# swacisko/ALGA

Measured on AMD Instinct MI355X. Metric: overlap_edges_per_sec, higher is better.
Workload: dtype u32; 1 GPU; cfg4_50M_150bp: 50000000 x 150 bp reads, genome 250000000, seed 11, err 0.00 -> 90621096 nodes (both strands, duplicates removed), min_overlap 82, rsoemo 116; generated on the device (alga_amd.workload.device_build) in 1.0 s; nodes=90621096, edges=92350115

## Files before the change

### alga_amd/csrc/engine.hip

```cpp
#include <hip/hip_runtime.h>

#include <algorithm>
#include <chrono>
#include <cstdio>
#include <cstdlib>
#include <cstring>
#include <new>
#include <string>
#include <thread>
#include <vector>

#include "engine_internal.h"

using namespace alga;

namespace {

using Prepared = AlgaPrepared;

int prepare(alga_engine *e, const alga_nodes *nodes, const alga_prefsuf_params *p, hipStream_t s, Prepared &out) {
    if (!nodes || !p) return alga_fail(e, ALGA_ERR_INVALID_ARGUMENT, "nodes/params must not be NULL");
    if (nodes->n < 0) return alga_fail(e, ALGA_ERR_INVALID_ARGUMENT, "negative node count");
    if (nodes->n > 0 && (!nodes->words || !nodes->len)) return alga_fail(e, ALGA_ERR_INVALID_ARGUMENT, "words/len must not be NULL");
    if (nodes->stride_words <= 0 && nodes->n > 0) return alga_fail(e, ALGA_ERR_INVALID_ARGUMENT, "stride_words must be positive");
// ... 417 lines not shown
                            (unsigned long long *) e->seg_val.p, n_rec, bits, s));
    launch_rowptr_from_sorted((const uint32_t *) e->seg_key.p, cnt + CNT_SORT_VALID, n_rec, n_owned, (uint32_t *) e->rowptr.p, s);
    if ((rc = alga_check_launch(e, "k_rowptr_from_sorted"))) return rc;
    launch_gather_heads(nd, (const unsigned long long *) e->seg_val.p, cnt + CNT_SORT_VALID, n_rec, e->heads.p, s);
    if ((rc = alga_check_launch(e, "k_gather_heads"))) return rc;
    HIP_TRY(e, hipEventRecord(e->ev[EV_GROUP], s));

    if ((rc = alga_ensure(e, e->out_cnt, (size_t) (n_owned + 1) * sizeof(uint32_t)))) return rc;
    if ((rc = alga_ensure(e, e->outdeg, (size_t) (nd.n + 1) * sizeof(uint32_t)))) return rc;
    HIP_TRY(e, hipMemsetAsync(e->outdeg.p, 0, (size_t) (nd.n + 1) * sizeof(uint32_t), s));
    const int tpb = reduce_targets_per_block(n_valid_hint, (uint64_t) std::max(1, n_owned));
    launch_reduce_targets(nd, cfg, dst_begin, n_owned, tpb, (const uint32_t *) e->rowptr.p, (unsigned long long *) e->seg_val.p,
                          e->heads.p, (uint32_t *) e->out_cnt.p, (uint32_t *) e->outdeg.p, cnt, s);
    if ((rc = alga_check_launch(e, "k_reduce_targets"))) return rc;
    HIP_TRY(e, hipEventRecord(e->ev[EV_REDUCE], s));

    if ((rc = alga_ensure(e, e->scan_scratch, scan_scratch_bytes((uint64_t) nd.n)))) return rc;
    if ((rc = alga_ensure(e, e->out_rowptr, (size_t) (nd.n + 1) * sizeof(uint32_t)))) return rc;
    launch_exclusive_scan((const uint32_t *) e->outdeg.p, (uint64_t) nd.n, (uint32_t *) e->out_rowptr.p, (uint64_t *) e->scan_scratch.p, s);
    if ((rc = alga_check_launch(e, "scan(outdeg)"))) return rc;
    uint64_t *d_total = (uint64_t *) e->scan_scratch.p + scan_total_index((uint64_t) nd.n);
    HIP_TRY(e, hipMemcpyAsync(&e->h_counters[CNT_TOTAL], d_total, sizeof(uint64_t), hipMemcpyDeviceToHost, s));
    HIP_TRY(e, hipMemcpyAsync(e->h_counters, cnt, CNT_TOTAL * sizeof(unsigned long long), hipMemcpyDeviceToHost, s));
    HIP_TRY(e, hipStreamSynchronize(s));
    const uint64_t E = e->h_counters[CNT_TOTAL];
    if (E >= (1ull << 32) - 16) return alga_fail(e, ALGA_ERR_CAPACITY, "more than 2^32 edges; shard the input");
    if ((rc = alga_ensure(e, e->edges, (size_t) (E + 1) * sizeof(alga_edge_dev)))) return rc;
    launch_scatter_by_source(cfg, dst_begin, n_owned, (const uint32_t *) e->rowptr.p, (const unsigned long long *) e->seg_val.p,
                             (const uint32_t *) e->out_cnt.p, (const uint32_t *) e->out_rowptr.p, (uint32_t *) e->outdeg.p,
                             (alga_edge_dev *) e->edges.p, s);
    if ((rc = alga_check_launch(e, "k_scatter_by_source"))) return rc;
    launch_sort_rows(nd.n, (const uint32_t *) e->out_rowptr.p, (alga_edge_dev *) e->edges.p, s);
    if ((rc = alga_check_launch(e, "k_sort_rows"))) return rc;
    HIP_TRY(e, hipEventRecord(e->ev[EV_EMIT], s));
    HIP_TRY(e, hipStreamSynchronize(s));
    *n_edges = E;
    e->stats.edges = E;
    e->stats.transitive_listed = e->h_counters[CNT_TR_LISTED];
    e->stats.transitive_compares = e->h_counters[CNT_TR_COMPARES];
    e->stats.transitive_removed = e->h_counters[CNT_TR_REMOVED];
    e->stats.max_in_records = e->h_counters[CNT_MAX_IN];
    return ALGA_OK;
}

int finalize_local(alga_engine *e, const Prepared &pp, int32_t src_begin, int32_t src_end, uint64_t n_rec, hipStream_t s, uint64_t *n_edges) {
    int rc;
    *n_edges = 0;
    const uint64_t n_src = (uint64_t) std::max<int64_t>(0, (int64_t) src_end - src_begin);
    if ((rc = alga_ensure(e, e->scan_scratch, scan_scratch_bytes(n_src)))) return rc;
    if ((rc = alga_ensure(e, e->out_rowptr, (size_t) (n_src + 1) * sizeof(uint32_t)))) return rc;
    if ((rc = alga_ensure(e, e->out_cnt, (size_t) (n_src + 1) * sizeof(uint32_t)))) return rc;
    HIP_TRY(e, hipEventRecord(e->ev[EV_GROUP], s));
    HIP_TRY(e, hipEventRecord(e->ev[EV_REDUCE], s));
    if (e->pile_deg_pending)
        launch_exclusive_scan_pile_deg((uint32_t *) e->outdeg.p, n_src, (uint32_t *) e->out_rowptr.p, (uint64_t *) e->scan_scratch.p, (unsigned long long *) e->loc_first.p,
                                       (const unsigned long long *) e->cl_pile_cnt.p, s);
    else
        launch_exclusive_scan((const uint32_t *) e->outdeg.p, n_src, (uint32_t *) e->out_rowptr.p, (uint64_t *) e->scan_scratch.p, s);
    e->pile_deg_pending = false;
    if ((rc = alga_check_launch(e, "scan(outdeg)"))) return rc;
    const uint64_t E = e->stats.records;
    if (E >= (1ull << 32) - 16) return alga_fail(e, ALGA_ERR_CAPACITY, "more than 2^32 edges; shard the input");
    if ((rc = alga_ensure(e, e->edges, (size_t) (E + 1) * sizeof(alga_edge_dev)))) return rc;
    launch_local_emit(src_begin, (int32_t) n_src, (const uint32_t *) e->outdeg.p, (const unsigned long long *) e->loc_first.p,
                      e->loc_second_used ? (const unsigned long long *) e->loc_second.p : nullptr, (const uint32_t *) e->rec_dst.p, (const unsigned long long *) e->rec_val.p, n_rec, (const uint32_t *) e->out_rowptr.p,
                      (uint32_t *) e->out_cnt.p, (alga_edge_dev *) e->edges.p,
                      e->defer_list_valid ? (const int32_t *) e->cl_defer.p : nullptr, (const unsigned long long *) e->counters.p + CNT_DEFERRED, (uint32_t) n_src, s,
                      e->loc_second_used ? e->loc_slot_stride : 0u);
    if ((rc = alga_check_launch(e, "k_local_emit"))) return rc;
    HIP_TRY(e, hipEventRecord(e->ev[EV_EMIT], s));
    uint64_t *d_total = (uint64_t *) e->scan_scratch.p + scan_total_index(n_src);
    HIP_TRY(e, hipMemcpyAsync(&e->h_counters[CNT_TOTAL], d_total, sizeof(uint64_t), hipMemcpyDeviceToHost, s));
    HIP_TRY(e, hipStreamSynchronize(s));
    if (e->h_counters[CNT_TOTAL] != E) return alga_fail(e, ALGA_ERR_HIP, "source-side emit: out-degrees and edge count disagree");
    *n_edges = E;
    e->stats.edges = E;
    return ALGA_OK;
}

int build_local(alga_engine *e, const Prepared &pp, int32_t src_begin, int32_t src_end, hipStream_t s, uint64_t *n_edges) {
    if (!pp.local_ok) return alga_fail(e, ALGA_ERR_UNSUPPORTED, "source-side reduction is not exact for this input (read lengths / masks / rsoemo)");
    uint64_t n_rec = 0;
    bool overflow = false;
    int rc = discover_impl(e, pp, src_begin, src_end, s, &n_rec, true, &overflow);
    if (rc) return rc;
    if (overflow) return alga_fail(e, ALGA_ERR_UNSUPPORTED, "a source node has more raw overlaps than the source-side reduction holds");
    if ((rc = finalize_local(e, pp, src_begin, src_end, n_rec, s, n_edges))) return rc;
    e->stats.reduction_used = ALGA_REDUCTION_SOURCE_SIDE;
    return ALGA_OK;
}

double now_ms_host() { return std::chrono::duration<double, std::milli>(std::chrono::steady_clock::now().time_since_epoch()).count(); }

float ev_ms(alga_engine *e, int a, int b) {
    float ms = 0.f;
    if (hipEventElapsedTime(&ms, e->ev[a], e->ev[b]) != hipSuccess) return 0.f;
    return ms;
}

void store_phase_stats(alga_engine *e) {
    if (!e->store_timed) return;
    e->stats.ms_keys = ev_ms(e, EV_START, EV_KEYS);
    e->stats.ms_sort = ev_ms(e, EV_KEYS, EV_SORT);
    e->stats.ms_dir = ev_ms(e, e->dir_late ? EV_SAMPLE : EV_SORT, EV_DIR);
    e->stats.ms_gather = ev_ms(e, EV_DIR, EV_GATHER) + (e->dir_late ? ev_ms(e, EV_SORT, EV_SAMPLE) : 0.0);
    e->stats.ms_pile = e->pile_timed ? ev_ms(e, EV_GATHER, EV_SEED) : 0.0;
}

}

int alga_prepare(alga_engine *e, const alga_nodes *nodes, const alga_prefsuf_params *p, hipStream_t s, AlgaPrepared &out) { return prepare(e, nodes, p, s, out); }
int alga_cluster_alloc(alga_engine *e, const AlgaPrepared &pp) { return cluster_alloc(e, pp); }

extern "C" {

int alga_abi_version(void) { return ALGA_AMD_ABI_VERSION; }

struct DeviceGuard {
    int prev = -1;
    DeviceGuard() { if (hipGetDevice(&prev) != hipSuccess) prev = -1; }
    ~DeviceGuard() { if (prev >= 0) (void) hipSetDevice(prev); }
// ... 38 lines not shown
    if (rc != ALGA_OK) { engine_free_handles(e); delete e; return rc; }
    *out = e;
    return ALGA_OK;
}

void alga_engine_destroy(alga_engine *e) {
    if (!e) return;
    DeviceGuard guard;
    (void) hipSetDevice(e->device);
    if (e->own_stream) (void) hipStreamSynchronize(e->own_stream);
    if (e->side_stream) (void) hipStreamSynchronize(e->side_stream);
    for (DevBuf *b : e->owned) alga_release(*b);
    alga_release(e->up_raw);
    for (DevBuf *b : {&e->in_bytes[0], &e->in_bytes[1], &e->in_nl[0], &e->in_nl[1], &e->in_tiles, &e->in_tile_off}) alga_release(*b);
    for (DevBuf *b : {&e->sp_rowptr, &e->sp_sorted, &e->sp_list, &e->sp_cnt, &e->sp_orow, &e->sp_out, &e->sp_in}) alga_release(*b);
    alga_staging_release(e);
    for (void *&p : e->gfa_pin) { if (p) (void) hipHostFree(p); p = nullptr; }
    for (auto &kv : e->host_lists) free(kv.first);
    e->host_lists.clear();
    engine_free_handles(e);
    delete e;
}

const char *alga_last_error(const alga_engine *e) { return e ? e->err.c_str() : "no engine"; }

int alga_engine_device_name(const alga_engine *e, char *buf, size_t buflen) {
    if (!e || !buf || buflen == 0) return ALGA_ERR_INVALID_ARGUMENT;
    snprintf(buf, buflen, "%s", e->dev_name);
    return ALGA_OK;
}

int alga_engine_set_option(alga_engine *e, const char *name, int64_t value) {
    if (!e || !name) return ALGA_ERR_INVALID_ARGUMENT;
    e->err.clear();
    if (!strcmp(name, "probe")) {
        if (value < ALGA_PROBE_AUTO || value > ALGA_PROBE_CLUSTER) return alga_fail(e, ALGA_ERR_INVALID_ARGUMENT, "option probe: 0 auto, 1 table, 2 cluster");
        e->opt_probe = (int) value;
    } else if (!strcmp(name, "cluster_bucket_bias")) {
        if (value < -8 || value > 8) return alga_fail(e, ALGA_ERR_INVALID_ARGUMENT, "option cluster_bucket_bias: -8 .. 8");
        e->opt_cluster_bucket_bias = (int) value;
    } else if (!strcmp(name, "cluster_pairs")) {
        e->opt_cluster_pairs = value != 0;
    } else if (!strcmp(name, "pile")) {
        e->opt_pile = (value == 2 || value == 3) ? (int) value : (value != 0);
    } else if (!strcmp(name, "pile_runs")) {
        e->opt_pile_runs = value != 0;
    } else if (!strcmp(name, "pile_runs_list")) {
        e->opt_pile_runs_list = value != 0;
    } else if (!strcmp(name, "pile_dir")) {
        if (value < 0 || value > 2) return alga_fail(e, ALGA_ERR_INVALID_ARGUMENT, "option pile_dir: 0 directory records, 1 k_pile_build from the keys, 2 ... and no directory for a pure pile build");
        e->opt_pile_dir = (int) value;
    } else if (!strcmp(name, "pile_deg_fold")) {
        e->opt_pile_deg_fold = value != 0;
    } else if (!strcmp(name, "pile_probe_lean")) {
        e->opt_pile_probe_lean = value != 0;
    } else if (!strcmp(name, "pile_stream_by_id")) {
        e->opt_pile_stream_by_id = value != 0;
    } else if (!strcmp(name, "pile_check")) {
        e->opt_pile_check = value != 0;
    } else if (!strcmp(name, "pile_skip_gather")) {
        e->opt_pile_skip_gather = value != 0;
    } else if (!strcmp(name, "cluster_order")) {
        e->opt_cluster_order = value != 0;
    } else if (!strcmp(name, "local_big_max")) {
        e->big_limit = value < 0 ? -1 : (int) std::min<int64_t>(value, 1 << 20);
    } else if (!strcmp(name, "shard_bucket_max")) {
        e->opt_shard_dmax = (int) std::max<int64_t>(1, std::min<int64_t>(value, 4096));
    } else if (!strcmp(name, "rsort_variant")) {
        rsort_set_variant((int) value);
    } else if (!strcmp(name, "stream_slots")) {
        e->opt_stream_slots = value >= 4 ? 4 : 2;
    } else if (!strcmp(name, "pile_range")) {
        e->opt_pile_range = value != 0;
    } else if (!strcmp(name, "pkb_legacy")) {
        e->opt_pkb_legacy = (int) value;
    } else if (!strcmp(name, "own_sort")) {
        e->opt_own_sort = value != 0;
    } else if (!strcmp(name, "test_presort_oom")) {
        e->opt_test_presort_oom = value != 0;
    } else if (!strcmp(name, "test_pile_oom")) {
        e->opt_test_pile_oom = value != 0;
    } else if (!strcmp(name, "test_unsorted_index")) {
        e->opt_test_unsorted_index = value != 0;
    } else if (!strcmp(name, "gfa_chunk_mb")) {
        if (value < 1 || value > 4096) return alga_fail(e, ALGA_ERR_INVALID_ARGUMENT, "option gfa_chunk_mb: 1 .. 4096");
        e->opt_gfa_chunk_mb = (int) value;
    } else if (!strcmp(name, "mst_mid_nodes")) {
        if (value < 8 || value > (1 << 20)) return alga_fail(e, ALGA_ERR_INVALID_ARGUMENT, "option mst_mid_nodes: 8 .. 2^20");
        e->opt_mst_mid_nodes = (int) value;
    } else if (!strcmp(name, "consensus_max_blocks")) {
        if (value < 0 || value > (1 << 20)) return alga_fail(e, ALGA_ERR_INVALID_ARGUMENT, "option consensus_max_blocks: 0 .. 2^20");
        e->opt_consensus_max_blocks = (int) value;
    } else if (!strcmp(name, "unitig_ruling")) {
        if (value < -1 || value > 1) return alga_fail(e, ALGA_ERR_INVALID_ARGUMENT, "option unitig_ruling: -1, 0 or 1");
        e->opt_unitig_ruling = (int) value;
    } else if (!strcmp(name, "correct_slice_keys")) {
        if (value < 1 || value > (1ll << 31)) return alga_fail(e, ALGA_ERR_INVALID_ARGUMENT, "option correct_slice_keys: 1 .. 2^31");
        e->opt_correct_slice_keys = value;
    } else if (!strcmp(name, "correct_dir_bits")) {
        if (value < 0 || value > 28) return alga_fail(e, ALGA_ERR_INVALID_ARGUMENT, "option correct_dir_bits: 0 (auto) or 1 .. 28");
        e->opt_correct_dir_bits = (int) value;
    } else if (!strcmp(name, "place_dir_bits")) {
        if (value < 0 || value > 26) return alga_fail(e, ALGA_ERR_INVALID_ARGUMENT, "option place_dir_bits: 0 (auto) or 1 .. 26");
        e->opt_place_dir_bits = (int) value;
    } else if (!strcmp(name, "auto_reduction_per_target")) {
        e->opt_force_per_target = value != 0;
// ... 668 lines not shown
```

### alga_amd/csrc/engine_internal.h

```cpp
#pragma once
#include <hip/hip_runtime.h>

#include <cstdio>
#include <algorithm>
#include <string>
#include <vector>
#include <unordered_map>

#include "../../include/alga_amd.h"
#include "prefsuf_common.h"
#include "prefsuf_kernels.h"
#include "pkb_kernels.h"

struct DevBuf {
    void  *p = nullptr;
    size_t cap = 0;
};

enum { EV_START = 0, EV_SEED, EV_PROBE, EV_GROUP, EV_REDUCE, EV_EMIT, EV_PAIRS, EV_KEYS, EV_SORT, EV_GATHER, EV_DIR, EV_SAMPLE, EV_COUNT };
constexpr int ALGA_STAGE_THREADS = 8;

struct alga_engine {
    std::vector<DevBuf *> owned;
    int         device = -1;
    hipStream_t own_stream = nullptr;
    hipStream_t side_stream = nullptr;
    hipEvent_t  ev_side = nullptr;
    std::string err;
    char        dev_name[256] = {0};
    int         n_cu = 256;
    int         seed_fill_x10 = 20;
    int         opt_probe = 0;
    int         opt_cluster_bucket_bias = 0;
    int         opt_force_per_target = 0;
    int         opt_shard_dmax = 4096;
    int         opt_test_unsorted_index = 0;
    hipEvent_t  ev[EV_COUNT] = {};
    DevBuf table, filter, counters, rowptr, rec_dst, rec_val, keys, seg_key, seg_val, heads, sort_temp, out_cnt, outdeg, out_rowptr, edges, scan_scratch;
    DevBuf cl_defer;
    uint32_t h_first_hkey = 255;
    int32_t keyed_n = -1, keyed_begin = 0, keyed_end = 0;
    bool defer_list_valid = false;
    const void *keyed_words = nullptr;
    int32_t store_n = -1, store_run_begin = 0, store_run_end = 0, store_eq = 0;
    uint32_t store_buckets = 0;
    const void *store_words = nullptr;
    int stat_max_len = 0, stat_min_len = 0; uint64_t stat_live = 0; unsigned long long stat_mask_asym = 0;
    const void *stat_len = nullptr, *stat_from = nullptr, *stat_to = nullptr;
    bool   warmed = false;
    bool   pairs_timed = false;
    bool   store_timed = false;
    bool   pile_keys_only = false, pile_kept_pure = false;
    int    opt_pile_range = 1;
    int    opt_pile_skip_gather = 1;
    int    opt_pile = 1;
    int    opt_pile_runs = 1;
    int    opt_pile_runs_list = 1;
    DevBuf cl_pile_list;
    int    opt_pile_deg_fold = 1;
    int    opt_pile_dir = 2;
    bool   dir_late = false;
    bool   pile_tab_index = false;
    int    opt_pile_stream_by_id = 0;
    int    opt_pile_probe_lean = 1;
    bool   pile_deg_pending = false;
    int    opt_pile_check = 0;
    bool   expect_pairwise = false;
    DevBuf cl_pile_side_r, cl_pile_cursor;
    DevBuf cl_pile_own;
    int    opt_pkb_legacy = 0;
    int    opt_own_sort = 1;
    int    opt_test_presort_oom = 0;
    int    opt_test_pile_oom = 0;
    bool   pile_timed = false;
    DevBuf cl_pile_succ;
    DevBuf cl_pile_rec2;
    DevBuf cl_pile_rec, cl_pile_cnt, cl_pile_tab;
    uint32_t pile_epoch = 0;
    int32_t pile_n = -1; const void *pile_words = nullptr;
    int    opt_cluster_order = 1;
    int    opt_cluster_pairs = 1;
    DevBuf cl_keys[2], cl_vals[2], cl_meta, cl_runs, cl_nruns, cl_store, cl_dir;
    DevBuf loc_second;
    bool   loc_second_used = false;
    uint32_t loc_slot_stride = 0;
    int    opt_stream_slots = 4;
    DevBuf loc_first, loc_big_list, loc_big_items;
    int    big_limit = -1;
    DevBuf edge_keys, edge_keys2, edge_vals, edge_vals2, edges_sorted, xs_dst, xs_val;
    DevBuf up_words, up_len, up_from, up_to;
    DevBuf up_len_narrow;
    DevBuf cp_deg, cp_dst, cp_off;
    DevBuf cl_defer2;
    DevBuf pk_keys, pk_keys2, pk_vals, pk_vals2, pk_marks, pk_big, pk_add, pk_ekeys, pk_ekeys2, pk_flag, pk_pos, pk_edges[2], pk_rowptr, pk_deg,
           pk_mask, pk_cnt, pk_io, pk_io2, pk_tips, pk_heads, pk_g[2], pk_addk, pk_addk2, pk_merged, pk_hsz, pk_hsz2, pk_heads2, pk_nadd, pk_koff,
           pk_gsz, pk_fixlist, pk_bounds, pk_tiprec, pk_tipidx, pk_keys_all, pk_vals_all;
    DevBuf pk_keys2b, pk_vals2b, pk_headsb, pk_hszb, sort_temp2, pk_fixlist2, pk_cnt2;
    DevBuf pp_rows, pp_len, pp_perm[2], pp_keys[2], pp_mark, pp_keep, pp_pos, pp_out_rows, pp_out_len, pp_out_pair, pp_tally;
    bool        stage_ready = false;
    void       *stage_pin[ALGA_STAGE_THREADS][2] = {};
    hipEvent_t  stage_ev[ALGA_STAGE_THREADS][2] = {};
    hipStream_t stage_stream[ALGA_STAGE_THREADS] = {};
    DevBuf      up_raw;
    std::unordered_map<void *, size_t> host_lists;
    void       *host_spare = nullptr;
    size_t      host_spare_cap = 0;
    DevBuf      in_bytes[2], in_nl[2], in_tiles, in_tile_off;
    DevBuf      sp_rowptr, sp_sorted, sp_list, sp_cnt, sp_orow, sp_out, sp_in;
    DevBuf      tp_cnt, tp_keys[2], tp_vals[2], tp_flag, tp_pos, tp_best, tp_est, tp_rev, tp_rfid, tp_rowptr[2], tp_alive, tp_kill, tp_rec[2], tp_branch,
                tp_overflow, tp_ws, tp_out;
    DevBuf      mp_cnt, mp_rowptr, mp_rows, mp_len, mp_owner, mp_pend[2], mp_win, mp_overflow, mp_overflow2, mp_ws, mp_ws_big, mp_orow, mp_out;
    struct MstFilled { const void *p = nullptr; size_t bytes = 0; uint32_t hbits = 0, cap_nodes = 0, cap_edges = 0; int32_t n_ws = 0; } mp_filled[2];
// ... 195 lines not shown
```

### alga_amd/csrc/prefsuf_kernels.h

```cpp
#pragma once
#include <hip/hip_runtime.h>
#include <stddef.h>
#include <stdint.h>
#include "prefsuf_common.h"

namespace alga {

struct alga_edge_dev { int32_t src, dst, offset; };

void launch_restride(const uint32_t *in, int stride_in, uint32_t *out, int stride_out, uint64_t n, hipStream_t s);
void launch_widen_len(const void *in, int elem_bytes , int32_t *out, uint64_t n, hipStream_t s);
void launch_compact_edges(const alga_edge_dev *edges, int32_t n, uint64_t n_edges, uint8_t *deg, uint32_t *dst, uint8_t *off, unsigned long long *bad, hipStream_t s);
void launch_expand_twins(const uint32_t *in, int stride_in, const int32_t *len , uint32_t *out, int stride_out, uint64_t n_pairs, hipStream_t s);
void launch_node_stats(const NodesDev &nd, unsigned long long *counters, int *max_len , hipStream_t s);

uint32_t seed_buckets_for(uint64_t live_nodes, int fill_x10);
uint32_t seed_filter_bits_for(uint64_t live_nodes);
void launch_seed_build(const NodesDev &nd, const PrefSufCfg &cfg, unsigned long long *table, uint32_t n_buckets, uint32_t *filter,
                       uint32_t filter_bits, hipStream_t s);

struct ProbeBig { int32_t *list; uint32_t list_cap; uint32_t count; void *items; uint32_t item_cap; };
int    local_item_capacity();
int    local_big_limit();
size_t probe_big_bytes(int n_cu, uint32_t count, int local, uint32_t item_cap);

void launch_probe(const NodesDev &nd, const PrefSufCfg &cfg, const unsigned long long *table, uint32_t n_buckets,
                  const uint32_t *filter, uint32_t filter_bits, int32_t src_begin, int32_t src_end, uint32_t *rec_dst, unsigned long long *rec_val, uint64_t rec_cap,
                  unsigned long long *counters, int n_cu, int local , uint32_t *deg , unsigned long long *first ,
                  const ProbeBig *big , hipStream_t s);
uint64_t probe_record_slack(int n_cu, uint64_t n_src, bool local);
void launch_local_emit(int32_t src_base, int32_t n_src, const uint32_t *deg, const unsigned long long *first, const unsigned long long *second,
                       const uint32_t *rec_dst, const unsigned long long *rec_val, uint64_t n_rec, const uint32_t *rowptr, uint32_t *cursor,
                       alga_edge_dev *edges, const int32_t *record_sources, const unsigned long long *record_sources_count, uint32_t record_sources_cap, hipStream_t s, uint32_t slot_stride = 0);

bool       cluster_plan(const PrefSufCfg &cfg, int max_len, uint64_t live, int bucket_log2_bias, ClusterCfg *c, int *eq);
size_t     cluster_sort_temp_bytes(uint64_t n);
void       launch_cluster_keys(const NodesDev &nd, const PrefSufCfg &cfg, const ClusterCfg &cc, int32_t node_begin, int32_t node_end, uint32_t *keys,
                               uint32_t *vals, uint32_t *meta, void *runs, uint8_t *nruns, hipStream_t s, bool with_runs = true ,
                               const unsigned long long *only_if_declined = nullptr );
void       launch_cluster_runs_list(const NodesDev &nd, const PrefSufCfg &cfg, const ClusterCfg &cc, const int32_t *ids, const unsigned long long *count, uint32_t cap,
                                    uint32_t grid_blocks, void *runs, uint8_t *nruns, hipStream_t s);
hipError_t launch_cluster_store(const NodesDev &nd, const ClusterCfg &cc, uint32_t *keys, uint32_t *vals, uint32_t *keys2 , uint32_t *vals2, void *sort_temp,
                                size_t sort_temp_bytes, void *dir, bool fill_vals, hipEvent_t ev_sorted ,
                                unsigned long long *bad_flag ,
                                bool test_skip_sort , hipStream_t s, bool own_sort = true);
hipError_t launch_cluster_sort(const NodesDev &nd, const ClusterCfg &cc, uint32_t *keys, uint32_t *vals, uint32_t *keys2, uint32_t *vals2, void *sort_temp, size_t sort_temp_bytes,
                               bool fill_vals, hipEvent_t ev_sorted, bool test_skip_sort, hipStream_t s, bool own_sort = true);
hipError_t launch_cluster_dir(const NodesDev &nd, const ClusterCfg &cc, const uint32_t *keys2, void *dir, unsigned long long *bad_flag, const unsigned long long *only_if_no_pure_piles,
                              hipStream_t s);
hipError_t launch_cluster_gather(const NodesDev &nd, const ClusterCfg &cc, int eq, const uint32_t *keys2, const uint32_t *vals2, const uint32_t *meta,
                                 int uniform_len , void *store,
                                 const unsigned long long *pile_cnt , hipStream_t s);
uint64_t   cluster_record_slack(int n_cu, uint64_t n_src);
void       launch_probe_clustered(const NodesDev &nd, const PrefSufCfg &cfg, const ClusterCfg &cc, int eq, const void *store, const void *dir,
                                  const void *runs, const uint8_t *nruns, int32_t src_begin, int32_t src_end, const int32_t *src_list, int32_t src_base, uint32_t *rec_dst, unsigned long long *rec_val, uint64_t rec_cap,
                                  unsigned long long *counters, int n_cu, uint32_t *deg, unsigned long long *first, const ProbeBig *big,
                                  const unsigned long long *list_count ,
                                  int sw , hipStream_t s,
                                  const uint32_t *skeys = nullptr, const uint32_t *sids = nullptr, int uniform_len = 0,
                                  const unsigned long long *pile_cnt = nullptr ,
                                  const void *tab = nullptr , uint32_t epoch = 0);
void       launch_probe_stream(const NodesDev &nd, const PrefSufCfg &cfg, const ClusterCfg &cc, int eq, const void *store, const void *dir,
                               const void *runs, const uint8_t *nruns, int32_t src_begin, int32_t src_end, bool by_key ,
                               unsigned long long *counters, int n_cu, uint32_t *deg, unsigned long long *first, unsigned long long *second, int32_t *defer_list,
                               uint32_t defer_cap, const unsigned long long *pile_cnt ,
                               hipStream_t s, uint32_t slot_stride = 0 );
void       launch_pile_deg(int32_t n, unsigned long long *first, uint32_t *deg, const unsigned long long *pile_cnt, hipStream_t s);
bool       pile_plan(const PrefSufCfg &cfg, const ClusterCfg &cc, int eq, int uniform_len, bool masks);
size_t     pile_record_bytes(uint64_t n);
size_t     pile_table_bytes(uint32_t n_buckets);
void       launch_pile_sample(const NodesDev &nd, const ClusterCfg &cc, int uniform_len, const uint32_t *skeys , const uint32_t *sids , const void *dir,
                              unsigned long long *pile_cnt , int no_sample, hipStream_t s,
                              bool from_keys = false );
constexpr int PILE_CNT_WORDS = 6;
size_t     pile_own_mask_bytes(uint64_t n);
size_t     pile_list_bytes(uint64_t n);
void       launch_pile_build(const NodesDev &nd, const PrefSufCfg &cfg, const ClusterCfg &cc, int uniform_len, const uint32_t *skeys, const uint32_t *sids, const void *dir, void *rec,
                             void *rec2 , void *tab, uint32_t epoch, void *side, const void *runs, int nwin, const unsigned long long *pile_cnt,
                             uint32_t *own_mask ,
                             void *plist , hipStream_t s,
                             bool from_keys = false , unsigned long long *bad_flag = nullptr,
                             bool full_record = false );
void       launch_pile_own_ids(const uint32_t *own_mask, const uint32_t *sids, uint64_t n_entries, int32_t *list, uint32_t cap, unsigned long long *pile_cnt, hipStream_t s);
void       launch_pile_check(const void *side, uint64_t n_entries, uint32_t n_buckets, const void *tab, const void *rec2, uint32_t epoch, const void *runs, int n_nodes, int nwin,
                             unsigned long long *pile_cnt, hipStream_t s);
bool       launch_probe_stream_list(const NodesDev &nd, const PrefSufCfg &cfg, const ClusterCfg &cc, int eq, const void *store, const void *dir, const void *runs, const uint8_t *nruns,
// ... 67 lines not shown
```

### alga_amd/csrc/prefsuf_kernels.hip

```cpp
#include <hip/hip_runtime.h>
#include <algorithm>
#include "prefsuf_common.h"
#include "prefsuf_kernels.h"
#include "prefsuf_device.h"
#include "prefsuf_cluster_device.h"

namespace alga {

__global__ void __launch_bounds__(256) k_node_stats(NodesDev nd, unsigned long long *counters, int *max_len) {
    __shared__ int s_max[4], s_min[4];
    __shared__ unsigned long long s_live[4];
    int m = 0, mn = 0x7FFFFFFF;
    unsigned long long live = 0, asym = 0;
    auto one = [&](int l, int64_t i) {
        m = l > m ? l : m;
        mn = (l > 0 && l < mn) ? l : mn;
        live += l > 0;
        if (nd.to && l > 0 && !nd.to[i] && (nd.from == nullptr || nd.from[i])) asym++;
    };
    const int64_t gid = (int64_t) blockIdx.x * blockDim.x + threadIdx.x, gsz = (int64_t) gridDim.x * blockDim.x;
    int64_t done = 0;
    if ((reinterpret_cast<uintptr_t>(nd.len) & 15u) == 0) {
        const int64_t nq = (int64_t) nd.n >> 2;
        const int4 *len4 = reinterpret_cast<const int4 *>(nd.len);
// ... 834 lines not shown
            atomicMax(&counters[CNT_MAX_IN], (unsigned long long) mk);
        }
    }
}

__global__ void __launch_bounds__(256)
k_scatter_by_source(PrefSufCfg cfg, int32_t dst_begin, int32_t n_owned, const uint32_t *__restrict__ rowptr,
                    const unsigned long long *__restrict__ seg_val, const uint32_t *__restrict__ out_cnt,
                    const uint32_t *__restrict__ out_rowptr, uint32_t *__restrict__ out_cursor, alga_edge_dev *__restrict__ edges) {
    const int t = blockIdx.x * blockDim.x + threadIdx.x;
    if (t >= n_owned) return;
    const uint32_t beg = rowptr[t], cnt = out_cnt[t];
    const int C = dst_begin + t;
    for (uint32_t u = 0; u < cnt; u++) {
        const unsigned long long v = seg_val[beg + u];
        const int A = (int) (uint32_t) v;
        const int off = ol_off((uint32_t) (v >> 32));
        const int row = cfg.reversed ? C : A;
        const int col = cfg.reversed ? A : C;
        const uint32_t pos = out_rowptr[row] + (atomicSub(&out_cursor[row], 1u) - 1u);
        edges[pos].src = row; edges[pos].dst = col; edges[pos].offset = off;
    }
}

__global__ void __launch_bounds__(256)
k_sort_rows(int32_t n, const uint32_t *__restrict__ out_rowptr, alga_edge_dev *__restrict__ edges) {
    const int a = blockIdx.x * blockDim.x + threadIdx.x;
    if (a >= n) return;
    const uint32_t beg = out_rowptr[a], k = out_rowptr[a + 1] - beg;
    alga_edge_dev *e = edges + beg;
    for (uint32_t i = 1; i < k; i++) {
        const alga_edge_dev x = e[i];
        uint32_t j = i;
        while (j > 0 && (e[j - 1].dst > x.dst || (e[j - 1].dst == x.dst && e[j - 1].offset > x.offset))) { e[j] = e[j - 1]; j--; }
        e[j] = x;
    }
}

__global__ void __launch_bounds__(256) k_edges_to_keys(const alga_edge_dev *__restrict__ e, uint64_t n, unsigned long long *__restrict__ keys,
                                                        uint32_t *__restrict__ vals) {
    for (uint64_t i = (uint64_t) blockIdx.x * blockDim.x + threadIdx.x; i < n; i += (uint64_t) gridDim.x * blockDim.x) {
        keys[i] = ((unsigned long long) (uint32_t) e[i].src << 32) | (uint32_t) e[i].dst;
        vals[i] = (uint32_t) e[i].offset;
    }
}

__global__ void __launch_bounds__(256) k_keys_to_edges(const unsigned long long *__restrict__ keys, const uint32_t *__restrict__ vals, uint64_t n,
                                                        alga_edge_dev *__restrict__ e) {
    for (uint64_t i = (uint64_t) blockIdx.x * blockDim.x + threadIdx.x; i < n; i += (uint64_t) gridDim.x * blockDim.x) {
        e[i].src = (int32_t) (keys[i] >> 32); e[i].dst = (int32_t) (uint32_t) keys[i]; e[i].offset = (int32_t) vals[i];
    }
}

__global__ void __launch_bounds__(256) k_local_emit_first(int32_t src_base, int32_t n_src, const uint32_t *__restrict__ deg,
                                                           const unsigned long long *__restrict__ first, const unsigned long long *__restrict__ second,
                                                           const uint32_t *__restrict__ rowptr, alga_edge_dev *__restrict__ edges, uint32_t slot_stride) {
    const int i = blockIdx.x * blockDim.x + threadIdx.x;
    if (i >= n_src) return;
    const uint32_t dg = deg[i];
    if (dg == 0) return;
    const unsigned long long f = first[i];
    if (f == LOCAL_FIRST_NONE) return;
    alga_edge_dev e;
    e.src = src_base + i; e.dst = (int32_t) (uint32_t) (f >> 32); e.offset = (int32_t) (uint32_t) f;
    const uint32_t at = rowptr[i];
    edges[at] = e;
    if (dg >= 3u && dg <= (uint32_t) LOCAL_SLOTS_MAX && second != nullptr && slot_stride != 0u) {
        unsigned long long k[LOCAL_SLOTS_MAX];
        k[0] = f;
#pragma unroll
        for (int q = 1; q < LOCAL_SLOTS_MAX; q++) k[q] = (uint32_t) q < dg ? second[(size_t) (q - 1) * slot_stride + (size_t) i] : ~0ull;
#pragma unroll
        for (int a = 0; a < LOCAL_SLOTS_MAX; a++)
#pragma unroll
            for (int b = (a & 1); b + 1 < LOCAL_SLOTS_MAX; b += 2) { const unsigned long long lo = min(k[b], k[b + 1]), hi = max(k[b], k[b + 1]); k[b] = lo; k[b + 1] = hi; }
#pragma unroll
        for (int q = 0; q < LOCAL_SLOTS_MAX; q++)
            if ((uint32_t) q < dg) { alga_edge_dev x; x.src = src_base + i; x.dst = (int32_t) (uint32_t) (k[q] >> 32); x.offset = (int32_t) (uint32_t) k[q]; edges[at + q] = x; }
        return;
    }
    if (dg == 2u && second != nullptr) {
        const unsigned long long g = second[i];
        alga_edge_dev e2 = e;
        e2.dst = (int32_t) (uint32_t) (g >> 32); e2.offset = (int32_t) (uint32_t) g;
        if (e2.dst < e.dst || (e2.dst == e.dst && e2.offset < e.offset)) { edges[at] = e2; e2 = e; }
        edges[at + 1] = e2;
    }
}

__global__ void __launch_bounds__(256) k_zero_cursors_list(const int32_t *__restrict__ list, const unsigned long long *__restrict__ count, uint32_t cap, int32_t src_base,
                                                            uint32_t *__restrict__ cursor) {
    unsigned long long m = *count;
    if (m > (unsigned long long) cap) m = cap;
    for (unsigned long long q = (unsigned long long) blockIdx.x * blockDim.x + threadIdx.x; q < m; q += (unsigned long long) gridDim.x * blockDim.x) cursor[list[q] - src_base] = 0u;
}

__global__ void __launch_bounds__(256) k_sort_rows_list(const int32_t *__restrict__ list, const unsigned long long *__restrict__ count, uint32_t cap, int32_t src_base,
                                                         const uint32_t *__restrict__ out_rowptr, alga_edge_dev *__restrict__ edges) {
    unsigned long long m = *count;
    if (m > (unsigned long long) cap) m = cap;
    for (unsigned long long q = (unsigned long long) blockIdx.x * blockDim.x + threadIdx.x; q < m; q += (unsigned long long) gridDim.x * blockDim.x) {
        const int a = list[q] - src_base;
        const uint32_t beg = out_rowptr[a], k = out_rowptr[a + 1] - beg;
        alga_edge_dev *e = edges + beg;
        for (uint32_t i = 1; i < k; i++) {
            const alga_edge_dev x = e[i];
            uint32_t j = i;
            while (j > 0 && (e[j - 1].dst > x.dst || (e[j - 1].dst == x.dst && e[j - 1].offset > x.offset))) { e[j] = e[j - 1]; j--; }
            e[j] = x;
        }
    }
}

__global__ void __launch_bounds__(256) k_local_emit_records(int32_t src_base, const uint32_t *__restrict__ rec_dst,
                                                             const unsigned long long *__restrict__ rec_val, uint64_t n_rec,
                                                             const uint32_t *__restrict__ rowptr, uint32_t *__restrict__ cursor,
                                                             alga_edge_dev *__restrict__ edges) {
    for (uint64_t i = (uint64_t) blockIdx.x * blockDim.x + threadIdx.x; i < n_rec; i += (uint64_t) gridDim.x * blockDim.x) {
        const uint32_t c = rec_dst[i];
        if (c == REC_INVALID) continue;
        const unsigned long long v = rec_val[i];
        const int32_t src = (int32_t) (uint32_t) v;
        alga_edge_dev e;
        e.src = src; e.dst = (int32_t) c; e.offset = ol_off((uint32_t) (v >> 32));
        edges[rowptr[src - src_base] + atomicAdd(&cursor[src - src_base], 1u)] = e;
    }
}

__global__ void __launch_bounds__(256) k_restride(const uint32_t *__restrict__ in, int stride_in, uint32_t *__restrict__ out, int stride_out, uint64_t n) {
    const uint64_t total = n * (uint64_t) stride_out;
    for (uint64_t i = (uint64_t) blockIdx.x * blockDim.x + threadIdx.x; i < total; i += (uint64_t) gridDim.x * blockDim.x) {
        const uint64_t r = i / (uint64_t) stride_out;
        const int c = (int) (i - r * (uint64_t) stride_out);
        out[i] = c < stride_in ? in[r * (uint64_t) stride_in + c] : 0u;
    }
}

__device__ __forceinline__ uint32_t nuc_revcomp32(uint32_t x) {
    x = __brev(x);
    x = ((x >> 1) & 0x55555555u) | ((x & 0x55555555u) << 1);
// ... 116 lines not shown
struct ProbeTable { const unsigned long long *table; uint32_t n_buckets; const uint32_t *filter; uint32_t filter_mask; };

template <int NQ, int LOCAL>
static void launch_probe_nql(const NodesDev &nd, const PrefSufCfg &cfg, const ProbeTable &t,
                             int32_t src_begin, int32_t src_end, const ProbeOut &o, dim3 grid, dim3 block, hipStream_t s) {
    if constexpr (LOCAL != 0) {
        if (o.big_count) {
            hipLaunchKernelGGL((k_probe_sources<true, NQ, LOCAL, true>), grid, block, 0, s, nd, cfg, t.table, t.n_buckets, t.filter, t.filter_mask, src_begin, src_end, o);
            return;
        }
    }
    if (cfg.stats) hipLaunchKernelGGL((k_probe_sources<true, NQ, LOCAL>), grid, block, 0, s, nd, cfg, t.table, t.n_buckets, t.filter, t.filter_mask, src_begin, src_end, o);
    else           hipLaunchKernelGGL((k_probe_sources<false, NQ, LOCAL>), grid, block, 0, s, nd, cfg, t.table, t.n_buckets, t.filter, t.filter_mask, src_begin, src_end, o);
}
template <int NQ>
static void launch_probe_nq(const NodesDev &nd, const PrefSufCfg &cfg, const ProbeTable &t, int local,
                            int32_t src_begin, int32_t src_end, const ProbeOut &o, dim3 grid, dim3 block, hipStream_t s) {
    if (local == 1)      launch_probe_nql<NQ, 1>(nd, cfg, t, src_begin, src_end, o, grid, block, s);
    else if (local == 2) launch_probe_nql<NQ, 2>(nd, cfg, t, src_begin, src_end, o, grid, block, s);
    else                 launch_probe_nql<NQ, 0>(nd, cfg, t, src_begin, src_end, o, grid, block, s);
}

void launch_probe(const NodesDev &nd, const PrefSufCfg &cfg, const unsigned long long *table, uint32_t n_buckets,
                  const uint32_t *filter, uint32_t filter_bits,
                  int32_t src_begin, int32_t src_end, uint32_t *rec_dst, unsigned long long *rec_val, uint64_t rec_cap,
                  unsigned long long *counters, int n_cu, int local, uint32_t *deg, unsigned long long *first, const ProbeBig *big, hipStream_t s) {
    const int64_t ns = (int64_t) src_end - src_begin;
    if (ns <= 0) return;
    const bool second = local && big && big->count > 0;
    dim3 grid((unsigned) probe_blocks(n_cu, second ? (uint64_t) big->count : (uint64_t) ns)), block(PROBE_WAVES * 64);
    ProbeOut o{rec_dst, rec_val, rec_cap, counters, deg, first, src_begin};
    if (local && big) {
        o.big_list = big->list; o.big_list_cap = big->list_cap;
        if (second) {
            const size_t items = (size_t) grid.x * PROBE_WAVES * (size_t) big->item_cap;
            o.big_count = big->count;
            o.bigO = (uint4 *) big->items;
            o.bigC = (uint32_t *) (o.bigO + items * (size_t) local);
            o.bigM = o.bigC + items;
            o.big_cap = big->item_cap;
        }
    }
    ProbeTable t{table, n_buckets, filter_bits ? filter : nullptr, filter_bits ? filter_bits - 1 : 0u};
    const int need_q = (((2 * cfg.Lcap + 31) >> 5) + 3) >> 2;
    const bool aligned = (nd.stride & 3) == 0 && ((uintptr_t) nd.words & 15u) == 0;
    const int row_q = nd.stride >> 2;
    if (aligned && need_q <= 2 && row_q >= 2)      launch_probe_nq<2>(nd, cfg, t, local, src_begin, src_end, o, grid, block, s);
    else if (aligned && need_q <= 3 && row_q >= 3) launch_probe_nq<3>(nd, cfg, t, local, src_begin, src_end, o, grid, block, s);
    else if (aligned && need_q <= 4 && row_q >= 4) launch_probe_nq<4>(nd, cfg, t, local, src_begin, src_end, o, grid, block, s);
    else                                           launch_probe_nq<0>(nd, cfg, t, local, src_begin, src_end, o, grid, block, s);
}

void launch_local_emit(int32_t src_base, int32_t n_src, const uint32_t *deg, const unsigned long long *first, const unsigned long long *second,
                       const uint32_t *rec_dst, const unsigned long long *rec_val, uint64_t n_rec, const uint32_t *rowptr, uint32_t *cursor,
                       alga_edge_dev *edges, const int32_t *record_sources, const unsigned long long *record_sources_count, uint32_t record_sources_cap, hipStream_t s,
                       uint32_t slot_stride) {
    if (n_src <= 0) return;
    if (record_sources) hipLaunchKernelGGL(k_zero_cursors_list, dim3(std::min<unsigned>(grid_for((uint64_t) record_sources_cap, 256), 2048u)), dim3(256), 0, s, record_sources, record_sources_count,
                                           record_sources_cap, src_base, cursor);
    else (void) hipMemsetAsync(cursor, 0, (size_t) (n_src + 1) * sizeof(uint32_t), s);
    hipLaunchKernelGGL(k_local_emit_first, dim3(grid_for((uint64_t) n_src, 256)), dim3(256), 0, s, src_base, n_src, deg, first, second, rowptr, edges, slot_stride);
    if (n_rec) {
        unsigned g = std::min<unsigned>(grid_for(n_rec, 256), 4096u);
        hipLaunchKernelGGL(k_local_emit_records, dim3(std::max(1u, g)), dim3(256), 0, s, src_base, rec_dst, rec_val, n_rec, rowptr, cursor, edges);
    }
    if (record_sources) {
        if (n_rec) hipLaunchKernelGGL(k_sort_rows_list, dim3(std::min<unsigned>(grid_for((uint64_t) record_sources_cap, 256), 2048u)), dim3(256), 0, s, record_sources, record_sources_count,
                                      record_sources_cap, src_base, rowptr, edges);
    } else hipLaunchKernelGGL(k_sort_rows, dim3(grid_for((uint64_t) n_src, 256)), dim3(256), 0, s, n_src, rowptr, edges);
}

void launch_make_keys(const uint32_t *rec_dst, uint64_t n_rec, int32_t dst_begin, int32_t dst_end, uint32_t *keys,
                      unsigned long long *n_valid, hipStream_t s) {
    if (n_rec == 0) return;
    unsigned g = std::min<unsigned>(grid_for(n_rec, 256 * 4), 4096u);
    hipLaunchKernelGGL(k_make_keys, dim3(std::max(1u, g)), dim3(256), 0, s, rec_dst, n_rec, dst_begin, dst_end, keys, n_valid);
}

void launch_rowptr_from_sorted(const uint32_t *keys, const unsigned long long *n_valid_ptr, uint64_t n_rec_max, int32_t n_owned,
                               uint32_t *rowptr, hipStream_t s) {
    unsigned g = std::min<unsigned>(grid_for(n_rec_max + 1, 256), 8192u);
    hipLaunchKernelGGL(k_rowptr_from_sorted, dim3(std::max(1u, g)), dim3(256), 0, s, keys, n_valid_ptr, n_owned, rowptr);
}

size_t scan_scratch_bytes(uint64_t n) {
    uint64_t tiles = (n + SCAN_TILE - 1) / SCAN_TILE;
    return (size_t) (tiles + 2) * sizeof(uint64_t);
}

void launch_exclusive_scan(const uint32_t *in, uint64_t n, uint32_t *out, uint64_t *scratch, hipStream_t s) {
    if (n == 0) { (void) hipMemsetAsync(out, 0, sizeof(uint32_t), s); (void) hipMemsetAsync(scratch, 0, 2 * sizeof(uint64_t), s); return; }
    const uint32_t tiles = (uint32_t) ((n + SCAN_TILE - 1) / SCAN_TILE);
    hipLaunchKernelGGL(k_scan_tile_sums, dim3(tiles), dim3(SCAN_BLOCK), 0, s, in, n, scratch);
    hipLaunchKernelGGL(k_scan_spine, dim3(1), dim3(1024), 0, s, scratch, tiles);
    hipLaunchKernelGGL(k_scan_tiles, dim3(tiles), dim3(SCAN_BLOCK), 0, s, in, n, scratch, out);
}

void launch_exclusive_scan_pile_deg(uint32_t *deg, uint64_t n, uint32_t *out, uint64_t *scratch, unsigned long long *first, const unsigned long long *pile_cnt, hipStream_t s) {
    if (n == 0) { launch_exclusive_scan(deg, n, out, scratch, s); return; }
    const uint32_t tiles = (uint32_t) ((n + SCAN_TILE - 1) / SCAN_TILE);
    hipLaunchKernelGGL(k_scan_tile_sums_pile_deg, dim3(tiles), dim3(SCAN_BLOCK), 0, s, deg, n, scratch, first, pile_cnt);
    hipLaunchKernelGGL(k_scan_spine, dim3(1), dim3(1024), 0, s, scratch, tiles);
    hipLaunchKernelGGL(k_scan_tiles, dim3(tiles), dim3(SCAN_BLOCK), 0, s, (const uint32_t *) deg, n, scratch, out);
}

uint64_t scan_total_index(uint64_t n) { return (n + SCAN_TILE - 1) / SCAN_TILE; }

__global__ void __launch_bounds__(256) k_mail(MailArgs a, uint32_t *__restrict__ dst) {
    for (int i = 0; i < a.n; i++)
        for (uint32_t w = threadIdx.x; w < a.seg[i].words; w += 256) dst[a.seg[i].dst + w] = a.seg[i].src[w];
}

void launch_mail(const MailArgs &a, uint32_t *host_block_dev, hipStream_t s) {
    if (a.n > 0) hipLaunchKernelGGL(k_mail, dim3(1), dim3(256), 0, s, a, host_block_dev);
// ... 53 lines not shown
```

Measured before the change: 5.377 billion edges/s.

## Fuse out-degree exclusive scan with local edge emission in a tiled kernel

Replaces the separate exclusive scan of out-degrees followed by k_local_emit_first with a three-kernel sequence: per-tile degree sums (decoding piled degrees from the first slot), a single-block serial spine scan, and a tile kernel that computes row offsets and emits the first/slot edges in the same pass. This removes one full write-then-read of the rowptr array and the separate pile-degree fold pass over the loc_first array. The trade-off is a second read of deg/first in the tile-sum pass and a one-block spine scan, and the change adds a new default-on option with more complex degree decoding that must match the old pile_deg scan.

```diff
diff --git a/alga_amd/csrc/engine.hip b/alga_amd/csrc/engine.hip
--- a/alga_amd/csrc/engine.hip
+++ b/alga_amd/csrc/engine.hip
@@ -493,21 +493,24 @@
     if ((rc = alga_ensure(e, e->out_cnt, (size_t) (n_src + 1) * sizeof(uint32_t)))) return rc;
     HIP_TRY(e, hipEventRecord(e->ev[EV_GROUP], s));
     HIP_TRY(e, hipEventRecord(e->ev[EV_REDUCE], s));
-    if (e->pile_deg_pending)
-        launch_exclusive_scan_pile_deg((uint32_t *) e->outdeg.p, n_src, (uint32_t *) e->out_rowptr.p, (uint64_t *) e->scan_scratch.p, (unsigned long long *) e->loc_first.p,
-                                       (const unsigned long long *) e->cl_pile_cnt.p, s);
-    else
-        launch_exclusive_scan((const uint32_t *) e->outdeg.p, n_src, (uint32_t *) e->out_rowptr.p, (uint64_t *) e->scan_scratch.p, s);
+    const bool fused = e->opt_emit_fused != 0;
+    const unsigned long long *pile_cnt = e->pile_deg_pending ? (const unsigned long long *) e->cl_pile_cnt.p : nullptr;
+    if (!fused) {
+        if (e->pile_deg_pending)
+            launch_exclusive_scan_pile_deg((uint32_t *) e->outdeg.p, n_src, (uint32_t *) e->out_rowptr.p, (uint64_t *) e->scan_scratch.p, (unsigned long long *) e->loc_first.p, pile_cnt, s);
+        else
+            launch_exclusive_scan((const uint32_t *) e->outdeg.p, n_src, (uint32_t *) e->out_rowptr.p, (uint64_t *) e->scan_scratch.p, s);
+        if ((rc = alga_check_launch(e, "scan(outdeg)"))) return rc;
+    }
     e->pile_deg_pending = false;
-    if ((rc = alga_check_launch(e, "scan(outdeg)"))) return rc;
     const uint64_t E = e->stats.records;
     if (E >= (1ull << 32) - 16) return alga_fail(e, ALGA_ERR_CAPACITY, "more than 2^32 edges; shard the input");
     if ((rc = alga_ensure(e, e->edges, (size_t) (E + 1) * sizeof(alga_edge_dev)))) return rc;
     launch_local_emit(src_begin, (int32_t) n_src, (const uint32_t *) e->outdeg.p, (const unsigned long long *) e->loc_first.p,
-                      e->loc_second_used ? (const unsigned long long *) e->loc_second.p : nullptr, (const uint32_t *) e->rec_dst.p, (const unsigned long long *) e->rec_val.p, n_rec, (const uint32_t *) e->out_rowptr.p,
+                      e->loc_second_used ? (const unsigned long long *) e->loc_second.p : nullptr, (const uint32_t *) e->rec_dst.p, (const unsigned long long *) e->rec_val.p, n_rec, (uint32_t *) e->out_rowptr.p,
                       (uint32_t *) e->out_cnt.p, (alga_edge_dev *) e->edges.p,
                       e->defer_list_valid ? (const int32_t *) e->cl_defer.p : nullptr, (const unsigned long long *) e->counters.p + CNT_DEFERRED, (uint32_t) n_src, s,
-                      e->loc_second_used ? e->loc_slot_stride : 0u);
+                      e->loc_second_used ? e->loc_slot_stride : 0u, fused ? (uint64_t *) e->scan_scratch.p : nullptr, fused ? pile_cnt : nullptr);
     if ((rc = alga_check_launch(e, "k_local_emit"))) return rc;
     HIP_TRY(e, hipEventRecord(e->ev[EV_EMIT], s));
     uint64_t *d_total = (uint64_t *) e->scan_scratch.p + scan_total_index(n_src);
@@ -652,6 +655,8 @@
         e->opt_pile_dir = (int) value;
     } else if (!strcmp(name, "pile_deg_fold")) {
         e->opt_pile_deg_fold = value != 0;
+    } else if (!strcmp(name, "emit_fused")) {
+        e->opt_emit_fused = value != 0;
     } else if (!strcmp(name, "pile_probe_lean")) {
         e->opt_pile_probe_lean = value != 0;
     } else if (!strcmp(name, "pile_stream_by_id")) {
diff --git a/alga_amd/csrc/engine_internal.h b/alga_amd/csrc/engine_internal.h
--- a/alga_amd/csrc/engine_internal.h
+++ b/alga_amd/csrc/engine_internal.h
@@ -58,6 +58,7 @@
     int    opt_pile_runs_list = 1;
     DevBuf cl_pile_list;
     int    opt_pile_deg_fold = 1;
+    int    opt_emit_fused = 1;
     int    opt_pile_dir = 2;
     bool   dir_late = false;
     bool   pile_tab_index = false;
diff --git a/alga_amd/csrc/prefsuf_kernels.h b/alga_amd/csrc/prefsuf_kernels.h
--- a/alga_amd/csrc/prefsuf_kernels.h
+++ b/alga_amd/csrc/prefsuf_kernels.h
@@ -30,8 +30,9 @@
                   const ProbeBig *big , hipStream_t s);
 uint64_t probe_record_slack(int n_cu, uint64_t n_src, bool local);
 void launch_local_emit(int32_t src_base, int32_t n_src, const uint32_t *deg, const unsigned long long *first, const unsigned long long *second,
-                       const uint32_t *rec_dst, const unsigned long long *rec_val, uint64_t n_rec, const uint32_t *rowptr, uint32_t *cursor,
-                       alga_edge_dev *edges, const int32_t *record_sources, const unsigned long long *record_sources_count, uint32_t record_sources_cap, hipStream_t s, uint32_t slot_stride = 0);
+                       const uint32_t *rec_dst, const unsigned long long *rec_val, uint64_t n_rec, uint32_t *rowptr, uint32_t *cursor,
+                       alga_edge_dev *edges, const int32_t *record_sources, const unsigned long long *record_sources_count, uint32_t record_sources_cap, hipStream_t s, uint32_t slot_stride = 0,
+                       uint64_t *fused_scratch = nullptr, const unsigned long long *pile_cnt = nullptr);
 
 bool       cluster_plan(const PrefSufCfg &cfg, int max_len, uint64_t live, int bucket_log2_bias, ClusterCfg *c, int *eq);
 size_t     cluster_sort_temp_bytes(uint64_t n);
diff --git a/alga_amd/csrc/prefsuf_kernels.hip b/alga_amd/csrc/prefsuf_kernels.hip
--- a/alga_amd/csrc/prefsuf_kernels.hip
+++ b/alga_amd/csrc/prefsuf_kernels.hip
@@ -910,6 +910,34 @@
     }
 }
 
+__device__ __forceinline__ void local_emit_slots(int32_t src, size_t i, uint32_t dg, unsigned long long f, const unsigned long long *__restrict__ second,
+                                                 uint32_t at, alga_edge_dev *__restrict__ edges, uint32_t slot_stride) {
+    alga_edge_dev e;
+    e.src = src; e.dst = (int32_t) (uint32_t) (f >> 32); e.offset = (int32_t) (uint32_t) f;
+    edges[at] = e;
+    if (dg >= 3u && dg <= (uint32_t) LOCAL_SLOTS_MAX && second != nullptr && slot_stride != 0u) {
+        unsigned long long k[LOCAL_SLOTS_MAX];
+        k[0] = f;
+#pragma unroll
+        for (int q = 1; q < LOCAL_SLOTS_MAX; q++) k[q] = (uint32_t) q < dg ? second[(size_t) (q - 1) * slot_stride + i] : ~0ull;
+#pragma unroll
+        for (int a = 0; a < LOCAL_SLOTS_MAX; a++)
+#pragma unroll
+            for (int b = (a & 1); b + 1 < LOCAL_SLOTS_MAX; b += 2) { const unsigned long long lo = min(k[b], k[b + 1]), hi = max(k[b], k[b + 1]); k[b] = lo; k[b + 1] = hi; }
+#pragma unroll
+        for (int q = 0; q < LOCAL_SLOTS_MAX; q++)
+            if ((uint32_t) q < dg) { alga_edge_dev x; x.src = src; x.dst = (int32_t) (uint32_t) (k[q] >> 32); x.offset = (int32_t) (uint32_t) k[q]; edges[at + q] = x; }
+        return;
+    }
+    if (dg == 2u && second != nullptr) {
+        const unsigned long long g = second[i];
+        alga_edge_dev e2 = e;
+        e2.dst = (int32_t) (uint32_t) (g >> 32); e2.offset = (int32_t) (uint32_t) g;
+        if (e2.dst < e.dst || (e2.dst == e.dst && e2.offset < e.offset)) { edges[at] = e2; e2 = e; }
+        edges[at + 1] = e2;
+    }
+}
+
 __global__ void __launch_bounds__(256) k_local_emit_first(int32_t src_base, int32_t n_src, const uint32_t *__restrict__ deg,
                                                            const unsigned long long *__restrict__ first, const unsigned long long *__restrict__ second,
                                                            const uint32_t *__restrict__ rowptr, alga_edge_dev *__restrict__ edges, uint32_t slot_stride) {
@@ -919,31 +947,108 @@
     if (dg == 0) return;
     const unsigned long long f = first[i];
     if (f == LOCAL_FIRST_NONE) return;
-    alga_edge_dev e;
-    e.src = src_base + i; e.dst = (int32_t) (uint32_t) (f >> 32); e.offset = (int32_t) (uint32_t) f;
-    const uint32_t at = rowptr[i];
-    edges[at] = e;
-    if (dg >= 3u && dg <= (uint32_t) LOCAL_SLOTS_MAX && second != nullptr && slot_stride != 0u) {
-        unsigned long long k[LOCAL_SLOTS_MAX];
-        k[0] = f;
-#pragma unroll
-        for (int q = 1; q < LOCAL_SLOTS_MAX; q++) k[q] = (uint32_t) q < dg ? second[(size_t) (q - 1) * slot_stride + (size_t) i] : ~0ull;
-#pragma unroll
-        for (int a = 0; a < LOCAL_SLOTS_MAX; a++)
-#pragma unroll
-            for (int b = (a & 1); b + 1 < LOCAL_SLOTS_MAX; b += 2) { const unsigned long long lo = min(k[b], k[b + 1]), hi = max(k[b], k[b + 1]); k[b] = lo; k[b + 1] = hi; }
-#pragma unroll
-        for (int q = 0; q < LOCAL_SLOTS_MAX; q++)
-            if ((uint32_t) q < dg) { alga_edge_dev x; x.src = src_base + i; x.dst = (int32_t) (uint32_t) (k[q] >> 32); x.offset = (int32_t) (uint32_t) k[q]; edges[at + q] = x; }
-        return;
-    }
-    if (dg == 2u && second != nullptr) {
-        const unsigned long long g = second[i];
-        alga_edge_dev e2 = e;
-        e2.dst = (int32_t) (uint32_t) (g >> 32); e2.offset = (int32_t) (uint32_t) g;
-        if (e2.dst < e.dst || (e2.dst == e.dst && e2.offset < e.offset)) { edges[at] = e2; e2 = e; }
-        edges[at + 1] = e2;
-    }
+    local_emit_slots(src_base + i, (size_t) i, dg, f, second, rowptr[i], edges, slot_stride);
+}
+
+__device__ __forceinline__ uint32_t source_degree(uint32_t dg, bool piled, unsigned long long f) {
+    if (dg != 0u) return dg;
+    if (!piled || f == LOCAL_FIRST_NONE) return 0u;
+    return 1u + (uint32_t) ((f >> 8) & 1ull);
+}
+
+__global__ void __launch_bounds__(SCAN_BLOCK) k_emit_tile_sums(const uint32_t *__restrict__ deg, const unsigned long long *__restrict__ first, uint64_t n,
+                                                                const unsigned long long *__restrict__ pile_cnt, uint64_t *__restrict__ tile_sums) {
+    __shared__ uint32_t lds[8];
+    const bool piled = pile_cnt != nullptr && !pile_cnt_declines(pile_cnt);
+    const uint64_t base = (uint64_t) blockIdx.x * SCAN_TILE;
+    uint32_t s = 0;
+    if (base + SCAN_TILE <= n && (reinterpret_cast<uintptr_t>(deg) & 15u) == 0 && (reinterpret_cast<uintptr_t>(first) & 15u) == 0) {
+        constexpr int G = SCAN_ITEMS / 4;
+        const uint4 *d4 = reinterpret_cast<const uint4 *>(deg + base);
+        const ulonglong2 *f2 = reinterpret_cast<const ulonglong2 *>(first + base);
+        uint4 v[G];
+#pragma unroll
+        for (int k = 0; k < G; k++) v[k] = d4[k * SCAN_BLOCK + threadIdx.x];
+#pragma unroll
+        for (int k = 0; k < G; k++) {
+            const int g = 2 * (k * SCAN_BLOCK + (int) threadIdx.x);
+            ulonglong2 a = make_ulonglong2(LOCAL_FIRST_NONE, LOCAL_FIRST_NONE), b = a;
+            if (piled && (v[k].x == 0u || v[k].y == 0u)) a = f2[g];
+            if (piled && (v[k].z == 0u || v[k].w == 0u)) b = f2[g + 1];
+            s += source_degree(v[k].x, piled, a.x) + source_degree(v[k].y, piled, a.y) + source_degree(v[k].z, piled, b.x) + source_degree(v[k].w, piled, b.y);
+        }
+    } else {
+        for (int k = 0; k < SCAN_ITEMS; k++) {
+            const uint64_t i = base + (uint64_t) k * SCAN_BLOCK + threadIdx.x;
+            if (i < n) { const uint32_t dg = deg[i]; s += source_degree(dg, piled, (piled && dg == 0u) ? first[i] : LOCAL_FIRST_NONE); }
+        }
+    }
+    uint32_t tot;
+    block_exclusive_scan(s, &tot, lds);
+    if (threadIdx.x == 0) tile_sums[blockIdx.x] = tot;
+}
+
+__global__ void __launch_bounds__(1024) k_scan_spine_serial(uint64_t *tile_sums, uint32_t n_tiles) {
+    __shared__ uint64_t lds[16];
+    const int lane = lane_id(), wave = (int) (threadIdx.x >> 6);
+    const uint64_t per = ((uint64_t) n_tiles + 1023u) / 1024u;
+    const uint64_t beg = min((uint64_t) threadIdx.x * per, (uint64_t) n_tiles), end = min(beg + per, (uint64_t) n_tiles);
+    uint64_t sum = 0;
+    for (uint64_t i = beg; i < end; i++) sum += tile_sums[i];
+    uint64_t inc = sum;
+#pragma unroll
+    for (int o = 1; o < 64; o <<= 1) {
+        const uint32_t lo = (uint32_t) __shfl_up((int) (uint32_t) inc, o), hi = (uint32_t) __shfl_up((int) (uint32_t) (inc >> 32), o);
+        if (lane >= o) inc += ((uint64_t) hi << 32) | lo;
+    }
+    if (lane == 63) lds[wave] = inc;
+    __syncthreads();
+    uint64_t run = inc - sum;
+    for (int w = 0; w < wave; w++) run += lds[w];
+    for (uint64_t i = beg; i < end; i++) { const uint64_t v = tile_sums[i]; tile_sums[i] = run; run += v; }
+    if (threadIdx.x == 1023) tile_sums[n_tiles] = run;
+}
+
+__global__ void __launch_bounds__(SCAN_BLOCK) k_emit_scan_tiles(int32_t src_base, uint64_t n, const uint32_t *__restrict__ deg, const unsigned long long *__restrict__ first,
+                                                                 const unsigned long long *__restrict__ second, const unsigned long long *__restrict__ pile_cnt,
+                                                                 const uint64_t *__restrict__ tile_sums, uint32_t *__restrict__ out, alga_edge_dev *__restrict__ edges,
+                                                                 uint32_t slot_stride) {
+    __shared__ uint32_t lds[8];
+    const bool piled = pile_cnt != nullptr && !pile_cnt_declines(pile_cnt);
+    const int lane = lane_id(), wave = (int) (threadIdx.x >> 6);
+    const uint64_t wbase = (uint64_t) blockIdx.x * SCAN_TILE + (uint64_t) wave * (64 * SCAN_ITEMS) + (uint64_t) lane;
+    uint32_t d[SCAN_ITEMS];
+    unsigned long long f[SCAN_ITEMS];
+#pragma unroll
+    for (int k = 0; k < SCAN_ITEMS; k++) { const uint64_t i = wbase + 64u * k; d[k] = i < n ? deg[i] : 0u; }
+#pragma unroll
+    for (int k = 0; k < SCAN_ITEMS; k++) { const uint64_t i = wbase + 64u * k; f[k] = (i < n && (piled || d[k] != 0u)) ? first[i] : LOCAL_FIRST_NONE; }
+    uint32_t sum = 0;
+#pragma unroll
+    for (int k = 0; k < SCAN_ITEMS; k++) {
+        const uint32_t dk = source_degree(d[k], piled, f[k]);
+        if (d[k] == 0u && dk != 0u) f[k] &= 0xFFFFFFFF000000FFull;
+        d[k] = dk; sum += dk;
+    }
+    sum = (uint32_t) wave_sum_u64(sum);
+    if (lane == 0) lds[wave] = sum;
+    __syncthreads();
+    uint32_t run = (uint32_t) tile_sums[blockIdx.x];
+    for (int w = 0; w < wave; w++) run += lds[w];
+#pragma unroll
+    for (int k = 0; k < SCAN_ITEMS; k++) {
+        const uint64_t i = wbase + 64u * k;
+        uint32_t inc = d[k];
+#pragma unroll
+        for (int o = 1; o < 64; o <<= 1) { const uint32_t t = (uint32_t) __shfl_up((int) inc, o); if (lane >= o) inc += t; }
+        const uint32_t at = run + inc - d[k];
+        run += (uint32_t) __shfl((int) inc, 63);
+        if (i < n) {
+            out[i] = at;
+            if (d[k] != 0u && f[k] != LOCAL_FIRST_NONE) local_emit_slots(src_base + (int32_t) i, (size_t) i, d[k], f[k], second, at, edges, slot_stride);
+        }
+    }
+    if (blockIdx.x == gridDim.x - 1 && threadIdx.x == 0) out[n] = (uint32_t) tile_sums[gridDim.x];
 }
 
 __global__ void __launch_bounds__(256) k_zero_cursors_list(const int32_t *__restrict__ list, const unsigned long long *__restrict__ count, uint32_t cap, int32_t src_base,
@@ -1166,14 +1271,23 @@
 }
 
 void launch_local_emit(int32_t src_base, int32_t n_src, const uint32_t *deg, const unsigned long long *first, const unsigned long long *second,
-                       const uint32_t *rec_dst, const unsigned long long *rec_val, uint64_t n_rec, const uint32_t *rowptr, uint32_t *cursor,
+                       const uint32_t *rec_dst, const unsigned long long *rec_val, uint64_t n_rec, uint32_t *rowptr, uint32_t *cursor,
                        alga_edge_dev *edges, const int32_t *record_sources, const unsigned long long *record_sources_count, uint32_t record_sources_cap, hipStream_t s,
-                       uint32_t slot_stride) {
-    if (n_src <= 0) return;
+                       uint32_t slot_stride, uint64_t *fused_scratch, const unsigned long long *pile_cnt) {
+    if (n_src <= 0) {
+        if (fused_scratch) launch_exclusive_scan(deg, 0, rowptr, fused_scratch, s);
+        return;
+    }
     if (record_sources) hipLaunchKernelGGL(k_zero_cursors_list, dim3(std::min<unsigned>(grid_for((uint64_t) record_sources_cap, 256), 2048u)), dim3(256), 0, s, record_sources, record_sources_count,
                                            record_sources_cap, src_base, cursor);
     else (void) hipMemsetAsync(cursor, 0, (size_t) (n_src + 1) * sizeof(uint32_t), s);
-    hipLaunchKernelGGL(k_local_emit_first, dim3(grid_for((uint64_t) n_src, 256)), dim3(256), 0, s, src_base, n_src, deg, first, second, rowptr, edges, slot_stride);
+    if (fused_scratch) {
+        const uint32_t tiles = (uint32_t) (((uint64_t) n_src + SCAN_TILE - 1) / SCAN_TILE);
+        hipLaunchKernelGGL(k_emit_tile_sums, dim3(tiles), dim3(SCAN_BLOCK), 0, s, deg, first, (uint64_t) n_src, pile_cnt, fused_scratch);
+        hipLaunchKernelGGL(k_scan_spine_serial, dim3(1), dim3(1024), 0, s, fused_scratch, tiles);
+        hipLaunchKernelGGL(k_emit_scan_tiles, dim3(tiles), dim3(SCAN_BLOCK), 0, s, src_base, (uint64_t) n_src, deg, first, second, pile_cnt, (const uint64_t *) fused_scratch, rowptr, edges,
+                           slot_stride);
+    } else hipLaunchKernelGGL(k_local_emit_first, dim3(grid_for((uint64_t) n_src, 256)), dim3(256), 0, s, src_base, n_src, deg, first, second, (const uint32_t *) rowptr, edges, slot_stride);
     if (n_rec) {
         unsigned g = std::min<unsigned>(grid_for(n_rec, 256), 4096u);
         hipLaunchKernelGGL(k_local_emit_records, dim3(std::max(1u, g)), dim3(256), 0, s, src_base, rec_dst, rec_val, n_rec, rowptr, cursor, edges);
```

Measured after the change: 5.462 billion edges/s, median of 6. Within noise of the previous version (+1.6%).
